# AILab-CVC/SEED-X

Hardware: AMD Instinct MI355X
Metric: end-to-end generations/sec (img-in -> txt + 1024px-img-out) (higher is better)
Workload: dtype fp16

## Files before the change

### include/seedx_hip.h

```cpp
#ifndef SEEDX_HIP_H
#define SEEDX_HIP_H
#include <stdint.h>
#ifdef __cplusplus
extern "C" {
#endif

#define SX_OK 0
#define SX_ERR_INVALID 1
#define SX_ERR_HIP 2

#define SX_F16 0
#define SX_BF16 1
#define SX_F32 2
#define SX_BF16X3 3
#define SX_F16X2 4
#define SX_FP8_E4M3 5
#define SX_FP4_E2M1 6
#define SX_TILED16 0x100

#define SX_ACT_NONE 0
#define SX_ACT_GELU 1
#define SX_ACT_SILU 2

#define SX_A_LINEAR 0
// ... 16 lines not shown
  int32_t bias2d_rows;
  int32_t dtype;
  int32_t out_dtype;
  int32_t act;
  int32_t glu;
  int32_t a_mode;
  int32_t B, Hin, Win, Cin, Hout, Wout;
  int32_t stride;
  int32_t upsample;
  int32_t ld_bias2d;
  int32_t pad_mode;
  int32_t a_planes;
} sx_gemm_args;
int sx_gemm(const sx_gemm_args* args, void* stream);
int sx_gemm_gn(const sx_gemm_args* args, double* stats, int groups, int rows_per_sample, int* fused_host, void* stream);
typedef struct sx_gemm_ln_args {
  void* x16_out;
  double* row_stats_out;
  const double* row_stats_in;
  const float* colsum;
  int32_t ld_x16;
  int32_t dim;
  float eps;
  int32_t reserved;
} sx_gemm_ln_args;
int sx_gemm_ln(const sx_gemm_args* args, const sx_gemm_ln_args* ln, void* stream);
int sx_gemm_force_tile(int cfg);
int sx_gemm_debug_stamps(void* buf);
int sx_gemm_pick_tile(int M, int N, int K, int glu, int conv);

typedef struct sx_gemv_args {
  const void* x;
  const void* W;
  void* y;
  const float* residual;
  int32_t M, N, K;
  int32_t dtype, out_dtype, act, glu;
  int32_t w_layout;
  int32_t x_layout;
// ... 262 lines not shown
```

### seed-x_amd/_lib.py

```python
import ctypes as C
import os

_HERE = os.path.dirname(os.path.abspath(__file__))
LIB_PATH = os.path.join(_HERE, "lib", "libseedx_hip.so")

SX_F16, SX_BF16, SX_F32 = 0, 1, 2
SX_BF16X3 = 3
SX_F16X2 = 4
SX_FP8_E4M3 = 5
SX_FP4_E2M1 = 6
SX_TILED16 = 0x100
SX_ACT_NONE, SX_ACT_GELU, SX_ACT_SILU = 0, 1, 2
SX_A_LINEAR, SX_A_CONV3X3 = 0, 1

c_i32, c_i64, c_f32, c_vp = C.c_int32, C.c_int64, C.c_float, C.c_void_p


class GemmArgs(C.Structure):
    _fields_ = [("A", c_vp), ("W", c_vp), ("C", c_vp), ("bias", c_vp), ("bias2d", c_vp), ("residual", c_vp),
                ("M", c_i32), ("N", c_i32), ("K", c_i32), ("ldc", c_i32), ("ldr", c_i32), ("n_valid", c_i32),
                ("res_mod", c_i32), ("bias2d_rows", c_i32), ("dtype", c_i32), ("out_dtype", c_i32),
                ("act", c_i32), ("glu", c_i32), ("a_mode", c_i32),
                ("B", c_i32), ("Hin", c_i32), ("Win", c_i32), ("Cin", c_i32), ("Hout", c_i32), ("Wout", c_i32),
                ("stride", c_i32), ("upsample", c_i32), ("ld_bias2d", c_i32), ("pad_mode", c_i32), ("a_planes", c_i32)]


class GemmLnArgs(C.Structure):
    _fields_ = [("x16_out", c_vp), ("row_stats_out", c_vp), ("row_stats_in", c_vp), ("colsum", c_vp),
                ("ld_x16", c_i32), ("dim", c_i32), ("eps", c_f32), ("reserved", c_i32)]


class GemvArgs(C.Structure):
    _fields_ = [("x", c_vp), ("W", c_vp), ("y", c_vp), ("residual", c_vp),
                ("M", c_i32), ("N", c_i32), ("K", c_i32),
                ("dtype", c_i32), ("out_dtype", c_i32), ("act", c_i32), ("glu", c_i32),
                ("w_layout", c_i32), ("x_layout", c_i32), ("workspace", c_vp), ("workspace_bytes", C.c_uint64),
                ("x16_out", c_vp), ("row_ssq_out", c_vp), ("row_ssq_in", c_vp), ("ssq_in_parts", c_i32), ("ssq_dim", c_i32),
                ("ssq_eps", c_f32), ("x_planes", c_i32), ("out_planes", c_i32), ("x16_gamma", c_vp),
                ("w_dtype", c_i32), ("w_scale", c_vp), ("w_block_scale", c_vp),
                ("addend", c_vp), ("addend_sel", c_vp), ("addend_n", c_i32)]


class AttnF32Args(C.Structure):
    _fields_ = [("q", c_vp), ("kcache", c_vp), ("vcache", c_vp), ("out", c_vp), ("pos0_dev", c_vp),
# ... 168 lines not shown
```

### seed-x_amd/csrc/gemm.hip

```cpp
#include "gemm_common.h"

namespace sxk_gemm {

template <typename TT, int BM, int BN, int WM, int WN, int NSTAGE, int AMODE>
__global__ __launch_bounds__(WM * WN * 64) void gemm_kernel(const GemmP p) {
#if defined(__HIP_DEVICE_COMPILE__)
  typedef typename TT::vec8 vec8;
  constexpr int NW = WM * WN;
  static_assert(NW == 4 || NW == 8, "4 or 8 waves per block");
  constexpr int TM = BM / WM, TN = BN / WN;
  constexpr int FM = TM / 16, FN = TN / 16;
  constexpr bool kGlu = (FN % 2 == 0);
  constexpr int BNP = (BN + 8 * NW - 1) / (8 * NW) * (8 * NW);
  constexpr int A_PER_WAVE = BM / (8 * NW);
  constexpr int B_PER_WAVE = BNP / (8 * NW);
  constexpr int LOADS = A_PER_WAVE + B_PER_WAVE;
  constexpr int A_BYTES = BM * 128, B_BYTES = BNP * 128, STAGE = A_BYTES + B_BYTES;
  static_assert(LOADS * (NSTAGE - 1) <= 63, "vmcnt range");
  extern __shared__ __attribute__((aligned(16))) unsigned char smem[];

  const int tid = threadIdx.x, lane = tid & 63;
  const int wave = __builtin_amdgcn_readfirstlane(tid >> 6);
  const int wm = wave / WN, wn = wave % WN;
  unsigned long long t_start = 0, t_first = 0, t_main = 0;
// ... 364 lines not shown
  if (gn_fused) *gn_fused = 0;
  SX_CHECK(a->dtype == SX_F16 || a->dtype == SX_BF16, "sx_gemm: dtype must be f16/bf16");
  SX_CHECK(a->out_dtype >= SX_F16 && a->out_dtype <= SX_F32, "sx_gemm: bad out_dtype");
  SX_CHECK(a->M > 0 && a->N > 0 && a->K > 0, "sx_gemm: empty problem M=%d N=%d K=%d", a->M, a->N, a->K);
  SX_CHECK(a->K % 64 == 0, "sx_gemm: K=%d must be a multiple of 64 (pad the operand)", a->K);
  SX_CHECK(a->N % 16 == 0, "sx_gemm: N=%d must be a multiple of 16 (pad the weight)", a->N);
  SX_CHECK(!a->glu || a->N % 32 == 0, "sx_gemm: glu needs N %% 32 == 0");
  const int n_out = a->glu ? a->N / 2 : a->N;
  SX_CHECK(a->n_valid >= 0 && a->n_valid % 4 == 0 && a->n_valid <= n_out, "sx_gemm: n_valid=%d", a->n_valid);
  SX_CHECK(a->ldc >= (a->n_valid > 0 ? a->n_valid : n_out) && a->ldc % 4 == 0, "sx_gemm: ldc=%d invalid for n_out=%d",
           a->ldc, n_out);
  SX_CHECK(!a->residual || (a->ldr >= (a->n_valid > 0 ? a->n_valid : n_out) && a->ldr % 4 == 0), "sx_gemm: ldr=%d invalid", a->ldr);
  SX_CHECK(!a->bias2d || a->bias2d_rows > 0, "sx_gemm: bias2d_rows must be > 0");
  GemmP p;
  memset(&p, 0, sizeof(p));
  p.A = a->A; p.W = a->W; p.C = a->C; p.bias = a->bias; p.bias2d = a->bias2d; p.residual = a->residual;
  SX_CHECK(a->a_planes >= 0 && a->a_planes <= 2, "sx_gemm: a_planes=%d", a->a_planes);
  const int planes = a->a_planes == 2 ? 2 : 1;
  SX_CHECK(planes == 1 || (a->a_mode == SX_A_LINEAR && !ln), "sx_gemm: a_planes = 2 is for plain linear GEMMs");
  const int Kk = a->K * planes;
  p.M = a->M; p.N = a->N; p.K = Kk; p.Kw = a->K; p.ldc = a->ldc; p.ldr = a->ldr; p.res_mod = a->res_mod;
  p.n_valid = a->n_valid > 0 ? a->n_valid : n_out;
  p.bias2d_rows = a->bias2d_rows; p.out_dtype = a->out_dtype; p.act = a->act; p.glu = a->glu;
  p.ldb2 = a->ld_bias2d > 0 ? a->ld_bias2d : a->N;
  p.pad = 1;
  uint64_t a_bytes;
  if (a->a_mode == SX_A_CONV3X3) {
    SX_CHECK(a->Cin % 64 == 0 && a->K == 9 * a->Cin, "sx_gemm conv: Cin=%d K=%d", a->Cin, a->K);
    SX_CHECK(a->stride == 1 || a->stride == 2, "sx_gemm conv: stride");
    SX_CHECK(a->M == a->B * a->Hout * a->Wout, "sx_gemm conv: M != B*Hout*Wout");
// ... 17 lines not shown
  hipStream_t st = (hipStream_t)stream;
  p.res_init = (p.residual && p.act == SX_ACT_NONE && !p.glu) ? 1 : 0;
  if (ln) {
    SX_CHECK(a->a_mode == SX_A_LINEAR && !gn_stats, "sx_gemm_ln: linear GEMMs only");
    SX_CHECK(!(ln->row_stats_in && ln->row_stats_out), "sx_gemm_ln: a launch is a producer or a consumer, not both");
    if (ln->row_stats_out) {
      SX_CHECK(ln->x16_out && a->out_dtype == SX_F32 && !a->glu && a->act == SX_ACT_NONE && p.n_valid == a->N,
               "sx_gemm_ln producer: needs x16_out and a plain fp32 output of all N columns");
      SX_CHECK(ln->ld_x16 >= a->N && ln->ld_x16 % 4 == 0 && (((size_t)ln->x16_out) & 7) == 0, "sx_gemm_ln producer: ld_x16=%d", ln->ld_x16);
      p.ln_x16 = ln->x16_out; p.ln_ldx = ln->ld_x16; p.ln_out = ln->row_stats_out;
    } else {
      SX_CHECK(ln->colsum && ln->dim == a->K && ln->eps > 0.f, "sx_gemm_ln consumer: colsum / dim (= K) / eps");
      SX_CHECK(a->out_dtype == a->dtype && !a->residual && !a->bias2d, "sx_gemm_ln consumer: 16-bit output, no residual / bias2d");
      p.ln_in = ln->row_stats_in; p.ln_cs = ln->colsum; p.ln_eps = ln->eps; p.ln_inv_dim = 1.0f / (float)ln->dim;
    }
  }
  unsigned allow = 0x7f;
  if (ln) allow = 0;
  allow |= pp_supported(p, a->dtype, 256, a->a_mode) ? 0x80u : 0u;
  allow |= pp_supported(p, a->dtype, 320, a->a_mode) ? 0x100u : 0u;
  SX_CHECK(!(g_force_tile == 7 || g_force_tile == 8) || ((allow >> g_force_tile) & 1u),
           "sx_gemm: forced ping-pong tile has no kernel for this epilogue");
  if (ln) {
    const int plain = pick_tile(a->M, a->N, Kk, a->glu != 0, false, g_force_tile, 0x1ff);
    SX_CHECK((plain == 7 || plain == 8) && ((allow >> plain) & 1u),
             "sx_gemm_ln: M=%d N=%d K=%d does not run on a ping-pong tile with this epilogue (tile %d): keep sx_layernorm for it", a->M,
             a->N, a->K, plain);
    allow = 1u << plain;
  }
  const int cfg = pick_tile(a->M, a->N, Kk, a->glu != 0, a->a_mode == SX_A_CONV3X3, g_force_tile, allow);
  if (cfg == 7 || cfg == 8) {
    if (gn_stats && a->out_dtype == SX_F32 && !a->glu && a->act == SX_ACT_NONE && p.n_valid == a->N && a->N % gn_groups == 0 &&
        (a->N / gn_groups) % 2 == 0 && gn_rows % 256 == 0 && a->M % gn_rows == 0) {
      p.gn_stats = gn_stats; p.gn_groups = gn_groups; p.gn_cpg = a->N / gn_groups; p.gn_rows = gn_rows;
      *gn_fused = 1;
    }
    return launch_pp(p, a->dtype, cfg == 7 ? 256 : 320, a->a_mode, st);
  }
#define SX_GEMM_DISPATCH(TT)                                                  \
  switch (cfg) {                                                              \
    case 0: return launch_cfg<TT, 128, 128, 2, 2, 2>(p, a->a_mode, st);       \
    case 1: return launch_cfg<TT, 128, 80, 4, 1, 3>(p, a->a_mode, st);        \
    case 2: return launch_cfg<TT, 64, 128, 2, 2, 3>(p, a->a_mode, st);        \
    case 3: return launch_cfg<TT, 64, 64, 2, 2, 3>(p, a->a_mode, st);         \
    case 4: return launch_cfg<TT, 256, 256, 2, 4, 2>(p, a->a_mode, st);       \
    case 5: return launch_cfg<TT, 256, 320, 2, 4, 2>(p, a->a_mode, st);       \
    default: return launch_cfg<TT, 256, 160, 4, 2, 2>(p, a->a_mode, st);      \
  }
  if (a->dtype == SX_BF16) { SX_GEMM_DISPATCH(BF16) } else { SX_GEMM_DISPATCH(F16) }
#undef SX_GEMM_DISPATCH
}
```

### seed-x_amd/csrc/gemm_common.h

```cpp
#pragma once
#include "sx_common.h"

namespace sxk_gemm {

struct GemmP {
  const void* A;
  const void* W;
  void* C;
  const float* bias;
  const float* bias2d;
  const float* residual;
  int M, N, K, ldc, ldr, n_valid, res_mod, bias2d_rows, out_dtype, act, glu;
  int Kw;
  int Hin, Win, Cin, Hout, Wout, stride, upsample, ldb2, pad;
  int tiles_m, tiles_n, xm, xn;
  int gm;
  int res_init;
  unsigned a_bytes, w_bytes;
  unsigned long long* dbg;
  double* gn_stats;
  int gn_cpg, gn_groups, gn_rows;
  void* ln_x16;
  double* ln_out;
  const double* ln_in;
  const float* ln_cs;
  int ln_ldx;
  float ln_eps, ln_inv_dim;
};

template <int N>
__device__ __forceinline__ void wait_vmcnt() {
  asm volatile("s_waitcnt vmcnt(%0)" ::"n"(N) : "memory");
}

__device__ __forceinline__ bool tile_coords(const GemmP& p, int bid, int nblk, int& tile_m, int& tile_n) {
  if (p.xm == 0) {
    const int t = xcd_remap(bid, nblk);
    tile_m = t % p.tiles_m;
    tile_n = t / p.tiles_m;
    return true;
  }
  const int xcd = bid & 7, idx = bid >> 3;
// ... 21 lines not shown
    const double ab = (double)p.M * p.K, wb = (double)p.N * p.K;
    double best = 1e300;
    for (int xm = 1; xm <= 8; xm *= 2) {
      const int xn = 8 / xm;
      if (xm > p.tiles_m || xn > p.tiles_n) continue;
      const long padded = 8L * ((p.tiles_m + xm - 1) / xm) * ((p.tiles_n + xn - 1) / xn);
      const double cost = (ab * xn + wb * xm) * (1.0 + 4.0 * (double)(padded - grid) / grid);
      if (cost < best) { best = cost; p.xm = xm; p.xn = xn; }
    }
    if (p.xm) grid = 8 * ((p.tiles_m + p.xm - 1) / p.xm) * ((p.tiles_n + p.xn - 1) / p.xn);
    p.gm = gm_force > 0 ? gm_force : 8;
  }
  return grid;
}

int launch_pp(const GemmP& p, int dtype, int bn, int a_mode, hipStream_t st);
bool pp_supported(const GemmP& p, int dtype, int bn, int a_mode);

extern unsigned long long* g_dbg;
extern int g_gm;
extern int g_xcd_2d;

}
```

### seed-x_amd/csrc/gemm_pp.hip

```cpp
#include "gemm_common.h"
#include <type_traits>

namespace sxk_gemm {

#define SX_A_CONV3X3_UP 2

#define PP_SYNC()                            \
  do {                                       \
    __builtin_amdgcn_sched_barrier(0);       \
    __builtin_amdgcn_s_barrier();            \
    __builtin_amdgcn_sched_barrier(0);       \
  } while (0)

template <typename TT, int BN, int AMODE, bool OUT32, int ACT, bool GLU, int LN = 0>
__global__ __launch_bounds__(512) void gemm_pp_kernel(const GemmP p) {
#if defined(__HIP_DEVICE_COMPILE__)
  typedef typename TT::vec8 vec8;
  static_assert(LN != 2 || (OUT32 && !GLU && ACT == SX_ACT_NONE), "the LayerNorm producer is the plain fp32-output epilogue");
  constexpr int BM = 256, TN = BN / 4, FN = TN / 16, FM = 8, FH = 4;
  constexpr int NB = BN / 64;
  constexpr int C1 = NB - 3, C2 = 3;
  constexpr int WAITN = 4 + NB;
  constexpr int A_BYTES = BM * 128, STAGE = A_BYTES + BN * 128;
  static_assert(!GLU || FN % 2 == 0, "GLU pairs n-fragments");
  static_assert(BN == 256 || BN == 320, "ping-pong tiles are 256x256 and 256x320");
  extern __shared__ __attribute__((aligned(16))) unsigned char smem[];

  const int tid = threadIdx.x, lane = tid & 63;
  const int wave = __builtin_amdgcn_readfirstlane(tid >> 6);
  const int g = wave >> 2, wc = wave & 3;
// ... 199 lines not shown
    wait_vmcnt<WAITN>();
    lgkm0();
    PP_SYNC();
    mma(wf1, 1);
    PP_SYNC();
  };

  for (int kt = 0; kt < nkt; kt += 2) {
    ktile(std::integral_constant<int, 0>{}, kt);
    if (kt + 1 < nkt) ktile(std::integral_constant<int, 1>{}, kt + 1);
  }
  if (g == 0) PP_SYNC();
  wait_vmcnt<0>();

  if (p.dbg) t_main = __builtin_amdgcn_s_memtime();
  int ncol[FN], nout[FN];
  bool nok[FN];
  f32x4_t bv[FN];
#pragma unroll
  for (int i = 0; i < FN; ++i) {
    const int nb = n0 + wc * TN + i * 16;
    ncol[i] = nb + lq;
    nout[i] = GLU ? (nb >> 1) + lq : ncol[i];
    nok[i] = ncol[i] < p.N && nout[i] < p.n_valid && !(GLU && (i & 1));
    if (ncol[i] >= p.N) ncol[i] = p.N - 4;
    if (nout[i] + 4 > p.ldc) nout[i] = 0;
    bv[i] = (f32x4_t){0.f, 0.f, 0.f, 0.f};
  }
  if (p.bias) {
#pragma unroll
// ... 216 lines not shown
      for (int cp = c_lo >> 1; cp < (c_hi >> 1); ++cp) acc += gslot[((size_t)(BN / 2) + cp) * 2 + which];
      atomicAdd(&p.gn_stats[((size_t)smp * p.gn_groups + G) * 2 + which], (double)acc);
    }
  }
  if (p.dbg) {
    asm volatile("s_waitcnt vmcnt(0)" ::: "memory");
    const unsigned long long t_end = __builtin_amdgcn_s_memtime();
    if (tid == 0) {
      unsigned long long* d = p.dbg + (size_t)blockIdx.x * 4;
      d[0] = t_start; d[1] = t_first; d[2] = t_main; d[3] = t_end;
    }
  }
#endif
}

template <typename TT, int BN, int AMODE, bool OUT32, int ACT, bool GLU, int LN = 0>
static int launch_one(const GemmP& p0, hipStream_t st) {
  GemmP p = p0;
  p.dbg = g_dbg;
  const int grid = plan_grid(p, 256, BN, g_xcd_2d, g_gm);
  constexpr size_t lds = 2 * (size_t)(256 + BN) * 128 + (LN == 1 ? 2048 : 0);
  auto k = gemm_pp_kernel<TT, BN, AMODE, OUT32, ACT, GLU, LN>;
  static hipError_t attr[16];
  static bool done[16];
  int dev = 0;
  (void)hipGetDevice(&dev);
  dev &= 15;
  if (!done[dev]) {
    attr[dev] = hipFuncSetAttribute((const void*)k, hipFuncAttributeMaxDynamicSharedMemorySize, (int)lds);
    done[dev] = true;
  }
  SX_CHECK(attr[dev] == hipSuccess, "sx_gemm: cannot reserve %zu B of LDS for the 256x%d ping-pong tile: %s", lds, BN,
           hipGetErrorString(attr[dev]));
  hipLaunchKernelGGL(k, dim3(grid), dim3(512), lds, st, p);
  SX_HIP_LAUNCH_CHECK();
  return SX_OK;
}

static int epi_code(const GemmP& p, int dtype) {
  const bool out32 = p.out_dtype == SX_F32;
  if (!out32 && p.out_dtype != dtype) return -1;
  if (p.glu) {
    if (out32) return -1;
    if (p.act == SX_ACT_GELU) return 2;
    if (p.act == SX_ACT_SILU) return 3;
    return -1;
  }
  if (p.act == SX_ACT_NONE) return out32 ? 4 : 0;
  if (p.act == SX_ACT_GELU && !out32) return 1;
  return -1;
}

bool pp_supported(const GemmP& p, int dtype, int bn, int a_mode) {
  const int e = epi_code(p, dtype);
  if (e < 0) return false;
  if (p.ln_in && !(a_mode == SX_A_LINEAR && (e == 0 || e == 2) && !p.ln_out)) return false;
  if (p.ln_out && !(a_mode == SX_A_LINEAR && e == 4 && !p.gn_stats)) return false;
  if (bn == 320 && (e == 2 || e == 3)) return false;
  if (a_mode == SX_A_CONV3X3 && !(e == 0 || e == 4)) return false;
  if (a_mode == SX_A_CONV3X3 && p.upsample && !(p.stride == 1 && p.pad == 1)) return false;
  return bn == 256 || bn == 320;
}

template <typename TT>
static int launch_t(const GemmP& p, int dtype, int bn, int a_mode, hipStream_t st) {
  const int e = epi_code(p, dtype);
#define PP_CASE(BNV, AM, O32, ACTV, GLUV) return launch_one<TT, BNV, AM, O32, ACTV, GLUV>(p, st)
  if (p.ln_in) {
    if (e == 2) return launch_one<TT, 256, SX_A_LINEAR, false, SX_ACT_GELU, true, 1>(p, st);
    if (bn == 256) return launch_one<TT, 256, SX_A_LINEAR, false, SX_ACT_NONE, false, 1>(p, st);
    return launch_one<TT, 320, SX_A_LINEAR, false, SX_ACT_NONE, false, 1>(p, st);
  }
  if (p.ln_out) {
    if (bn == 256) return launch_one<TT, 256, SX_A_LINEAR, true, SX_ACT_NONE, false, 2>(p, st);
    return launch_one<TT, 320, SX_A_LINEAR, true, SX_ACT_NONE, false, 2>(p, st);
  }
  if (a_mode == SX_A_LINEAR) {
    if (bn == 256) {
      switch (e) {
        case 0: PP_CASE(256, SX_A_LINEAR, false, SX_ACT_NONE, false);
        case 1: PP_CASE(256, SX_A_LINEAR, false, SX_ACT_GELU, false);
        case 2: PP_CASE(256, SX_A_LINEAR, false, SX_ACT_GELU, true);
        case 3: PP_CASE(256, SX_A_LINEAR, false, SX_ACT_SILU, true);
        case 4: PP_CASE(256, SX_A_LINEAR, true, SX_ACT_NONE, false);
      }
// ... 21 lines not shown
      switch (e) {
        case 0: PP_CASE(256, SX_A_CONV3X3_UP, false, SX_ACT_NONE, false);
        case 4: PP_CASE(256, SX_A_CONV3X3_UP, true, SX_ACT_NONE, false);
      }
    } else {
      switch (e) {
        case 0: PP_CASE(320, SX_A_CONV3X3_UP, false, SX_ACT_NONE, false);
        case 4: PP_CASE(320, SX_A_CONV3X3_UP, true, SX_ACT_NONE, false);
      }
    }
  }
#undef PP_CASE
  return -1;
}

int launch_pp(const GemmP& p, int dtype, int bn, int a_mode, hipStream_t st) {
  if (!pp_supported(p, dtype, bn, a_mode)) return -1;
  return dtype == SX_BF16 ? launch_t<BF16>(p, dtype, bn, a_mode, st) : launch_t<F16>(p, dtype, bn, a_mode, st);
}

}
```

### seed-x_amd/ops.py

```python
import ctypes as C
import math

import os

import torch

from . import _lib
from ._lib import (SX_A_CONV3X3, SX_A_LINEAR, SX_ACT_GELU, SX_ACT_NONE, SX_ACT_SILU, SX_BF16, SX_F16, SX_F32,
                   AttnArgs, AttnSmallArgs, GemmArgs, GemvArgs, check)

_DT = {torch.float16: SX_F16, torch.bfloat16: SX_BF16, torch.float32: SX_F32}
_TD = {v: k for k, v in _DT.items()}
ACT = {None: SX_ACT_NONE, "none": SX_ACT_NONE, "gelu": SX_ACT_GELU, "silu": SX_ACT_SILU}


def dt_code(dtype):
    return _DT[dtype]


def _stream():
    return C.c_void_p(torch.cuda.current_stream().cuda_stream)


def _p(t):
# ... 34 lines not shown
def gemm_tile(M, N, K, glu=False, conv=False):
    return int(_lib.load().sx_gemm_pick_tile(int(M), int(N), int(K), 1 if glu else 0, 1 if conv else 0))


def ln_fold_ok(M, C, consumers, producers):
    return all(gemm_tile(M, n, C, glu) >= 7 for n, glu in consumers) and all(gemm_tile(M, C, k) >= 7 for k in producers)


def fold_layernorm(w, bias, gamma, beta):
    wf = (w.float() * gamma.float()[None, :]).to(w.dtype).contiguous()
    cs = wf.float().sum(dim=1).contiguous()
    b = w.float() @ beta.float()
    if bias is not None:
        b = b + bias.float()
    return wf, cs, b.contiguous()


GN_FUSE = os.environ.get("SX_GN_FUSE", "1") != "0"


def _launch_gemm(lib, args, gn, what):
    if gn is None or not GN_FUSE:
        check(lib.sx_gemm(C.byref(args), _stream()), what)
        return
    assert gn.buf.dtype == torch.float64 and gn.buf.is_contiguous() and args.M % gn.rows == 0 \
        and gn.buf.numel() == (args.M // gn.rows) * gn.groups * 2, "GnStats does not describe this output"
    fused = C.c_int32(0)
    check(lib.sx_gemm_gn(C.byref(args), gn.buf.data_ptr(), gn.groups, gn.rows, C.byref(fused), _stream()), what)
    gn.ready = bool(fused.value)


def gemm(a, w, bias=None, bias2d=None, bias2d_rows=0, residual=None, res_mod=0, act=None, glu=False,
         out_dtype=None, out=None, n_valid=0, ld_bias2d=0, gn=None, ln_emit=None, ln_apply=None, a_planes=1):
    lib = _lib.load()
    assert a.dim() == 2 and w.dim() == 2 and a.is_contiguous() and w.is_contiguous()
    assert a.dtype == w.dtype and a.dtype in (torch.float16, torch.bfloat16)
    M, K = a.shape
    N = w.shape[0]
    assert a_planes in (1, 2) and K % a_planes == 0
    K //= a_planes
    assert w.shape[1] == K, f"K mismatch {a.shape} vs {w.shape} (a_planes {a_planes})"
    n_out = N // 2 if glu else N
    n_store = n_valid if n_valid else n_out
    out_dtype = out_dtype or a.dtype
    if out is None:
        out = torch.empty((M, n_store), dtype=out_dtype, device=a.device)
    assert out.dtype == out_dtype and out.stride(-1) == 1 and out.shape[0] == M
    args = GemmArgs()
# ... 16 lines not shown
    args.out_dtype = _DT[out_dtype]
    args.act = ACT[act]
    args.glu = 1 if glu else 0
    args.a_mode = SX_A_LINEAR
    args.a_planes = a_planes
    if ln_emit is not None or ln_apply is not None:
        assert gn is None and not (ln_emit is not None and ln_apply is not None)
        la = _lib.GemmLnArgs()
        if ln_emit is not None:
            assert ln_emit.x16.shape == (M, N) and ln_emit.x16.dtype == a.dtype and ln_emit.stats.shape[0] == M
            la.x16_out, la.ld_x16, la.row_stats_out = ln_emit.x16.data_ptr(), ln_emit.x16.stride(0), ln_emit.stats.data_ptr()
        else:
            rows, colsum, eps = ln_apply
            assert rows.stats.shape[0] == M and colsum.dtype == torch.float32 and colsum.numel() == N and colsum.is_contiguous()
            la.row_stats_in, la.colsum, la.dim, la.eps = rows.stats.data_ptr(), colsum.data_ptr(), K, float(eps)
        check(lib.sx_gemm_ln(C.byref(args), C.byref(la), _stream()), "sx_gemm_ln")
        return out
    _launch_gemm(lib, args, gn, "sx_gemm")
    return out


def conv3x3(x, w, bias=None, bias2d=None, residual=None, stride=1, upsample=False, out_dtype=None, act=None,
            n_valid=0, pad_mode=0, gn=None):
    lib = _lib.load()
    assert x.dim() == 4 and x.is_contiguous() and w.is_contiguous()
    B, H, W, Cin = x.shape
    Cout, K = w.shape
    assert K == 9 * Cin
    hv, wv = (2 * H, 2 * W) if upsample else (H, W)
    padsum = 1 if pad_mode else 2
    Hout, Wout = (hv + padsum - 3) // stride + 1, (wv + padsum - 3) // stride + 1
    M = B * Hout * Wout
# ... 842 lines not shown
```

### seed-x_amd/unet.py

```python
import math
import os
import types

import torch

from . import ops
from .llama import glu_pack_rows

LN_FOLD = os.environ.get("SX_LN_FOLD", "1") != "0"

SDXL_BASE_CONFIG = dict(in_channels=4, out_channels=4, block_out_channels=(320, 640, 1280), layers_per_block=2,
                        down_attn=(False, True, True), up_attn=(True, True, False), transformer_layers=(1, 2, 10),
                        heads=(5, 10, 20), cross_attention_dim=2048, addition_time_embed_dim=256, pooled_dim=1280,
                        norm_groups=32, sample_size=128)


class UNetOutput:
    def __init__(self, sample):
        self.sample = sample


class UNet2DConditionModel:
    def __init__(self, comm=None, **cfg):
        from .parallel import Comm
# ... 133 lines not shown
                    wqkv=torch.cat([lin16(b + f".attn1.{q}.weight") for q in ("to_q", "to_k", "to_v")], 0).contiguous(),
                    wo1=lin16(b + ".attn1.to_out.0.weight"), bo1=f32(b + ".attn1.to_out.0.bias"),
                    n2=(f32(b + ".norm2.weight"), f32(b + ".norm2.bias")),
                    wq2=lin16(b + ".attn2.to_q.weight"),
                    wkv2=torch.cat([lin16(b + ".attn2.to_k.weight"), lin16(b + ".attn2.to_v.weight")], 0).contiguous(),
                    wo2=lin16(b + ".attn2.to_out.0.weight"), bo2=f32(b + ".attn2.to_out.0.bias"),
                    n3=(f32(b + ".norm3.weight"), f32(b + ".norm3.bias")),
                    wff1=glu_pack_rows(ffw[:half].contiguous(), ffw[half:].contiguous()),
                    bff1=glu_pack_rows(ffb[:half].reshape(-1, 1).contiguous(), ffb[half:].reshape(-1, 1).contiguous()).reshape(-1).contiguous(),
                    wff2=lin16(b + ".ff.net.2.weight"), bff2=f32(b + ".ff.net.2.bias")))
            if LN_FOLD:
                for blk in t["blocks"]:
                    blk["f1"] = ops.fold_layernorm(blk["wqkv"], None, *blk["n1"])
                    blk["f2"] = ops.fold_layernorm(blk["wq2"], None, *blk["n2"])
                    blk["f3"] = ops.fold_layernorm(blk["wff1"], blk["bff1"], *blk["n3"])
            self._xattn.append(t)
            return t

        self._temb_names, self._xattn = [], []
        boc = c["block_out_channels"]
        P = {}
        cin = c["in_channels"]
        self.cin_kpad = (9 * cin + 63) // 64 * 64
        w = sd["conv_in.weight"].detach().to(dev, dt).permute(0, 2, 3, 1).reshape(boc[0], -1)
        wp = torch.zeros(boc[0], self.cin_kpad, dtype=dt, device=dev)
        wp[:, :w.shape[1]] = w
        P["conv_in_w"], P["conv_in_b"] = wp, f32("conv_in.bias")
        P["te1"] = (lin16("time_embedding.linear_1.weight"), f32("time_embedding.linear_1.bias"))
        P["te2"] = (lin16("time_embedding.linear_2.weight"), f32("time_embedding.linear_2.bias"))
        P["ae1"] = (lin16("add_embedding.linear_1.weight"), f32("add_embedding.linear_1.bias"))
# ... 101 lines not shown
    def _transformer(self, t, x, B, ctx_kv, Hc, Wc, st_in=None):
        dt, heads = self.dtype, t["heads"]
        _, HW, C = x.shape
        hd = C // heads
        scale = hd ** -0.5
        sp = self.comm.world > 1
        h = self._gn(x, t["norm"], 1e-6, False, Hc, Wc, stats=st_in)
        nb = len(t["blocks"])
        M = B * HW
        if LN_FOLD and not sp and "f1" in t["blocks"][0] and self._ln_fold_ok(M, C):
            arena = torch.zeros((3 * nb, M, 2), dtype=torch.float64, device=x.device)

            def rows(i):
                return ops.LnRows(M, C, dt, x.device, stats=arena[i])
            ln = rows(0)
            hs = ops.gemm(h.view(-1, C), t["pin_w"], bias=t["pin_b"], out_dtype=torch.float32, ln_emit=ln)
            for k, b in enumerate(t["blocks"]):
                w, cs, bb = b["f1"]
                qkv = ops.gemm(ln.x16, w, bias=bb, ln_apply=(ln, cs, 1e-5)).view(B, HW, 3, heads, hd)
                att = ops.attention(qkv[:, :, 0], qkv[:, :, 1], qkv[:, :, 2], scale)
                ln = rows(3 * k + 1)
                hs = ops.gemm(att.view(-1, C), b["wo1"], bias=b["bo1"], residual=hs, out_dtype=torch.float32, ln_emit=ln)
                self._mark(hs)
                w, cs, bb = b["f2"]
                q = ops.gemm(ln.x16, w, bias=bb, ln_apply=(ln, cs, 1e-5)).view(B, HW, heads, hd)
                kv = ctx_kv[k]
                att = ops.attention(q, kv[:, :, 0], kv[:, :, 1], scale)
                ln = rows(3 * k + 2)
                hs = ops.gemm(att.view(-1, C), b["wo2"], bias=b["bo2"], residual=hs, out_dtype=torch.float32, ln_emit=ln)
                w, cs, bb = b["f3"]
                g = ops.gemm(ln.x16, w, bias=bb, act="gelu", glu=True, ln_apply=(ln, cs, 1e-5))
                if k == nb - 1:
                    hs = ops.gemm(g, b["wff2"], bias=b["bff2"], residual=hs, out_dtype=dt)
                else:
                    ln = rows(3 * k + 3)
                    hs = ops.gemm(g, b["wff2"], bias=b["bff2"], residual=hs, out_dtype=torch.float32, ln_emit=ln)
                self._mark(hs)
            st_out = self._gn_slot(B, HW)
            out = ops.gemm(hs, t["pout_w"], bias=t["pout_b"], residual=x.view(-1, C), out_dtype=torch.float32, gn=st_out)
            return out.view(B, HW, C), st_out
        hs = ops.gemm(h.view(-1, C), t["pin_w"], bias=t["pin_b"], out_dtype=torch.float32)
        for k, b in enumerate(t["blocks"]):
# ... 1 lines not shown
            if not sp:
                qkv = ops.gemm(n, b["wqkv"]).view(B, HW, 3, heads, hd)
                att = ops.attention(qkv[:, :, 0], qkv[:, :, 1], qkv[:, :, 2], scale)
            else:
                from . import seqpar
                kv_l = ops.gemm(n, b["wqkv"][C:]).view(B, HW, 2, heads, hd)
                pending = self.comm.all_gather_async(kv_l)
                q = ops.gemm(n, b["wqkv"][:C]).view(B, HW, heads, hd)
                g = pending.wait()
                kv = g.permute(1, 0, 2, 3, 4, 5).reshape(B, g.shape[0] * HW, 2, heads, hd).contiguous()
                att = ops.attention(q, kv[:, :, 0], kv[:, :, 1], scale)
            hs = ops.gemm(att.view(-1, C), b["wo1"], bias=b["bo1"], residual=hs, out_dtype=torch.float32)
            self._mark(hs)
            n = ops.layernorm(hs, b["n2"][0], b["n2"][1], 1e-5, dt)
            q = ops.gemm(n, b["wq2"]).view(B, HW, heads, hd)
            kv = ctx_kv[k]
            att = ops.attention(q, kv[:, :, 0], kv[:, :, 1], scale)
            hs = ops.gemm(att.view(-1, C), b["wo2"], bias=b["bo2"], residual=hs, out_dtype=torch.float32)
            n = ops.layernorm(hs, b["n3"][0], b["n3"][1], 1e-5, dt)
            g = ops.gemm(n, b["wff1"], bias=b["bff1"], act="gelu", glu=True)
            last = k == nb - 1
            hs = ops.gemm(g, b["wff2"], bias=b["bff2"], residual=hs, out_dtype=dt if last else torch.float32)
            self._mark(hs)
        st_out = self._gn_slot(B, HW)
        out = ops.gemm(hs, t["pout_w"], bias=t["pout_b"], residual=x.view(-1, C), out_dtype=torch.float32, gn=st_out)
        return out.view(B, HW, C), st_out

    def _ln_fold_ok(self, M, C):
        key = (M, C)
        if key not in self._ln_ok:
            self._ln_ok[key] = ops.ln_fold_ok(M, C, consumers=[(3 * C, False), (C, False), (8 * C, True)], producers=[C, 4 * C])
        return self._ln_ok[key]

    def prepare_context(self, encoder_hidden_states):
        P = self._pack()
        ehs = encoder_hidden_states
        key = (ehs.data_ptr(), ehs._version, tuple(ehs.shape))
        if self._ctx_key == key:
            return self._ctx
        B, L, ca = ehs.shape
        e16 = ops.cast(ehs.to(self.device).float().contiguous(), self.dtype).view(B * L, ca)
        ctx = []
        for t in self._xattn:
            heads = t["heads"]
            per = []
            for b in t["blocks"]:
                C = b["wq2"].shape[0]
                kv = ops.gemm(e16, b["wkv2"]).view(B, L, 2, heads, C // heads)
                per.append(kv)
            ctx.append(per)
        self._ctx_key, self._ctx = key, ctx
        return ctx

    def time_embeddings(self, t_vals, idx_dev, text_embeds, time_ids, B):
        P, dt, c = self._P, self.dtype, self.cfg
        boc0 = c["block_out_channels"][0]
        ts = ops.timestep_embedding(t_vals, boc0, dt, idx_dev=idx_dev, n=B)
        e = ops.gemm(ts, P["te1"][0], bias=P["te1"][1], act="silu")
        e = ops.gemm(e, P["te2"][0], bias=P["te2"][1], out_dtype=torch.float32)
        tid = ops.timestep_embedding(time_ids.reshape(-1).float().contiguous(), c["addition_time_embed_dim"], torch.float32)
        add = torch.empty((B, self.add_embedding.linear_1.in_features), dtype=torch.float32, device=self.device)
        ops.copy2d(text_embeds.float().contiguous(), add, 0)
        ops.copy2d(tid.view(B, -1), add, text_embeds.shape[1])
# ... 88 lines not shown
```

Baseline: 1.343.

## Fuse cross-attention into the LayerNorm-folded Q-projection GEMM epilogue

Adds an epilogue variant to the 320-wide ping-pong GEMM that, after computing the Q projection with folded LayerNorm, loads pre-packed K/V fragments for a 64-token context into LDS and runs softmax attention with MFMA directly on the register tile, writing the attention output. Q-projection weight columns are permuted so each wave owns whole heads (with a fifth head shared via LDS). Context K/V is additionally packed into an MFMA fragment layout once per context. This removes the Q write/read round trip and the separate attention launch per transformer block, at the cost of tight shape constraints (head_dim 64, 64 context tokens, heads multiple of 5) and heavier epilogue work per tile.

```diff
diff --git a/include/seedx_hip.h b/include/seedx_hip.h
--- a/include/seedx_hip.h
+++ b/include/seedx_hip.h
@@ -54,6 +54,15 @@
 } sx_gemm_args;
 int sx_gemm(const sx_gemm_args* args, void* stream);
 int sx_gemm_gn(const sx_gemm_args* args, double* stats, int groups, int rows_per_sample, int* fused_host, void* stream);
+typedef struct sx_xattn_args {
+  const void* kv_frag;
+  void* O;
+  int32_t heads, head_dim, skv;
+  int32_t rows_per_sample;
+  int32_t ld_o;
+  int32_t ld_kv;
+  float scale;
+} sx_xattn_args;
 typedef struct sx_gemm_ln_args {
   void* x16_out;
   double* row_stats_out;
@@ -63,6 +72,7 @@
   int32_t dim;
   float eps;
   int32_t reserved;
+  const void* xattn;
 } sx_gemm_ln_args;
 int sx_gemm_ln(const sx_gemm_args* args, const sx_gemm_ln_args* ln, void* stream);
 int sx_gemm_force_tile(int cfg);
diff --git a/seed-x_amd/_lib.py b/seed-x_amd/_lib.py
--- a/seed-x_amd/_lib.py
+++ b/seed-x_amd/_lib.py
@@ -25,9 +25,14 @@
                 ("stride", c_i32), ("upsample", c_i32), ("ld_bias2d", c_i32), ("pad_mode", c_i32), ("a_planes", c_i32)]
 
 
+class XattnArgs(C.Structure):
+    _fields_ = [("kv_frag", c_vp), ("O", c_vp), ("heads", c_i32), ("head_dim", c_i32), ("skv", c_i32),
+                ("rows_per_sample", c_i32), ("ld_o", c_i32), ("ld_kv", c_i32), ("scale", c_f32)]
+
+
 class GemmLnArgs(C.Structure):
     _fields_ = [("x16_out", c_vp), ("row_stats_out", c_vp), ("row_stats_in", c_vp), ("colsum", c_vp),
-                ("ld_x16", c_i32), ("dim", c_i32), ("eps", c_f32), ("reserved", c_i32)]
+                ("ld_x16", c_i32), ("dim", c_i32), ("eps", c_f32), ("reserved", c_i32), ("xattn", c_vp)]
 
 
 class GemvArgs(C.Structure):
diff --git a/seed-x_amd/csrc/gemm.hip b/seed-x_amd/csrc/gemm.hip
--- a/seed-x_amd/csrc/gemm.hip
+++ b/seed-x_amd/csrc/gemm.hip
@@ -402,6 +402,9 @@
   SX_CHECK(!a->bias2d || a->bias2d_rows > 0, "sx_gemm: bias2d_rows must be > 0");
   GemmP p;
   memset(&p, 0, sizeof(p));
+  XattnP xp;
+  const XattnP* xpp = nullptr;
+  memset(&xp, 0, sizeof(xp));
   p.A = a->A; p.W = a->W; p.C = a->C; p.bias = a->bias; p.bias2d = a->bias2d; p.residual = a->residual;
   SX_CHECK(a->a_planes >= 0 && a->a_planes <= 2, "sx_gemm: a_planes=%d", a->a_planes);
   const int planes = a->a_planes == 2 ? 2 : 1;
@@ -449,11 +452,30 @@
       SX_CHECK(a->out_dtype == a->dtype && !a->residual && !a->bias2d, "sx_gemm_ln consumer: 16-bit output, no residual / bias2d");
       p.ln_in = ln->row_stats_in; p.ln_cs = ln->colsum; p.ln_eps = ln->eps; p.ln_inv_dim = 1.0f / (float)ln->dim;
     }
+    if (const sx_xattn_args* xa = (const sx_xattn_args*)ln->xattn) {
+      SX_CHECK(ln->row_stats_in, "sx_gemm_ln: xattn rides on the consumer launch");
+      SX_CHECK(xa->kv_frag && xa->O && xa->scale > 0.f, "sx_gemm_ln xattn: kv_frag / O / scale");
+      SX_CHECK(xa->head_dim == 64 && xa->skv == 64, "sx_gemm_ln xattn: head_dim=%d skv=%d (64 / 64 only)", xa->head_dim, xa->skv);
+      SX_CHECK(xa->heads > 0 && xa->heads % 5 == 0 && a->N == 64 * xa->heads, "sx_gemm_ln xattn: heads=%d N=%d (heads %% 5 == 0, N = 64 heads)",
+               xa->heads, a->N);
+      SX_CHECK(xa->rows_per_sample > 0 && xa->rows_per_sample % 256 == 0 && a->M % xa->rows_per_sample == 0,
+               "sx_gemm_ln xattn: rows_per_sample=%d M=%d (whole 256-row tiles inside one sample)", xa->rows_per_sample, a->M);
+      SX_CHECK(a->act == SX_ACT_NONE && !a->glu && p.n_valid == a->N, "sx_gemm_ln xattn: plain projection only");
+      SX_CHECK(xa->ld_o >= a->N && xa->ld_o % 8 == 0 && (((size_t)xa->O) & 15) == 0 && (((size_t)xa->kv_frag) & 15) == 0,
+               "sx_gemm_ln xattn: ld_o=%d / alignment", xa->ld_o);
+      SX_CHECK(xa->ld_kv >= xa->heads * 8192 && xa->ld_kv % 8 == 0, "sx_gemm_ln xattn: ld_kv=%d", xa->ld_kv);
+      const uint64_t kv_bytes = (uint64_t)(a->M / xa->rows_per_sample - 1) * xa->ld_kv * 2ull + (uint64_t)xa->heads * 16384ull;
+      SX_CHECK(kv_bytes < 0x7fffffffull, "sx_gemm_ln xattn: packed K | V exceeds the 2 GiB descriptor range");
+      xp.kv = xa->kv_frag; xp.O = xa->O; xp.kv_bytes = (unsigned)kv_bytes; xp.heads = xa->heads;
+      xp.sample_bytes = (unsigned)xa->ld_kv * 2u;
+      xp.rows = xa->rows_per_sample; xp.ldo = xa->ld_o; xp.scale_log2 = xa->scale * 1.4426950408889634f;
+      xpp = &xp;
+    }
   }
   unsigned allow = 0x7f;
   if (ln) allow = 0;
-  allow |= pp_supported(p, a->dtype, 256, a->a_mode) ? 0x80u : 0u;
-  allow |= pp_supported(p, a->dtype, 320, a->a_mode) ? 0x100u : 0u;
+  allow |= pp_supported(p, a->dtype, 256, a->a_mode, xpp) ? 0x80u : 0u;
+  allow |= pp_supported(p, a->dtype, 320, a->a_mode, xpp) ? 0x100u : 0u;
   SX_CHECK(!(g_force_tile == 7 || g_force_tile == 8) || ((allow >> g_force_tile) & 1u),
            "sx_gemm: forced ping-pong tile has no kernel for this epilogue");
   if (ln) {
@@ -470,7 +492,7 @@
       p.gn_stats = gn_stats; p.gn_groups = gn_groups; p.gn_cpg = a->N / gn_groups; p.gn_rows = gn_rows;
       *gn_fused = 1;
     }
-    return launch_pp(p, a->dtype, cfg == 7 ? 256 : 320, a->a_mode, st);
+    return launch_pp(p, a->dtype, cfg == 7 ? 256 : 320, a->a_mode, st, xpp);
   }
 #define SX_GEMM_DISPATCH(TT)                                                  \
   switch (cfg) {                                                              \
diff --git a/seed-x_amd/csrc/gemm_common.h b/seed-x_amd/csrc/gemm_common.h
--- a/seed-x_amd/csrc/gemm_common.h
+++ b/seed-x_amd/csrc/gemm_common.h
@@ -26,6 +26,18 @@
   const float* ln_cs;
   int ln_ldx;
   float ln_eps, ln_inv_dim;
+};
+
+struct XattnP {
+  const void* kv;
+  void* O;
+  unsigned kv_bytes;
+  int heads, rows, ldo;
+  unsigned sample_bytes;
+  float scale_log2;
+};
+struct GemmPX : GemmP {
+  XattnP xa;
 };
 
 template <int N>
@@ -77,8 +89,8 @@
   return grid;
 }
 
-int launch_pp(const GemmP& p, int dtype, int bn, int a_mode, hipStream_t st);
-bool pp_supported(const GemmP& p, int dtype, int bn, int a_mode);
+int launch_pp(const GemmP& p, int dtype, int bn, int a_mode, hipStream_t st, const XattnP* xa = nullptr);
+bool pp_supported(const GemmP& p, int dtype, int bn, int a_mode, const XattnP* xa = nullptr);
 
 extern unsigned long long* g_dbg;
 extern int g_gm;
diff --git a/seed-x_amd/csrc/gemm_pp.hip b/seed-x_amd/csrc/gemm_pp.hip
--- a/seed-x_amd/csrc/gemm_pp.hip
+++ b/seed-x_amd/csrc/gemm_pp.hip
@@ -12,8 +12,8 @@
     __builtin_amdgcn_sched_barrier(0);       \
   } while (0)
 
-template <typename TT, int BN, int AMODE, bool OUT32, int ACT, bool GLU, int LN = 0>
-__global__ __launch_bounds__(512) void gemm_pp_kernel(const GemmP p) {
+template <typename TT, int BN, int AMODE, bool OUT32, int ACT, bool GLU, int LN = 0, bool XA = false>
+__global__ __launch_bounds__(512) void gemm_pp_kernel(const std::conditional_t<XA, GemmPX, GemmP> p) {
 #if defined(__HIP_DEVICE_COMPILE__)
   typedef typename TT::vec8 vec8;
   static_assert(LN != 2 || (OUT32 && !GLU && ACT == SX_ACT_NONE), "the LayerNorm producer is the plain fp32-output epilogue");
@@ -243,6 +243,154 @@
   wait_vmcnt<0>();
 
   if (p.dbg) t_main = __builtin_amdgcn_s_memtime();
+  if constexpr (XA) {
+    static_assert(BN == 320 && LN == 1 && !OUT32 && !GLU && ACT == SX_ACT_NONE && AMODE == SX_A_LINEAR, "cross-attention epilogue");
+    constexpr unsigned HEAD_B = 16384, Q5_OFF = 5 * HEAD_B, XB_OFF = Q5_OFF + 256 * 128, XC_OFF = XB_OFF + 2048;
+    static_assert(XC_OFF + 2048 <= 2 * STAGE, "K | V^T fragments, the fifth head's Q and the column vectors fit in the operand ring");
+    __syncthreads();
+    {
+      __amdgpu_buffer_rsrc_t rKV = __builtin_amdgcn_make_buffer_rsrc((void*)p.xa.kv, 0, (int)p.xa.kv_bytes, 0x00020000);
+      const unsigned kv0 = (unsigned)(m0 / p.xa.rows) * p.xa.sample_bytes + (unsigned)(5 * tile_n) * HEAD_B + (unsigned)lane * 16u;
+#pragma unroll
+      for (int i = 0; i < 10; ++i) {
+        const unsigned c = (unsigned)(wave * 10 + i) * 1024u;
+        __builtin_amdgcn_raw_ptr_buffer_load_lds(rKV, SX_LDS_PTR(smem + c), 16, kv0 + c, 0, 0, 0);
+      }
+      if (wave < 4) {
+        const float* src = wave < 2 ? p.bias : p.ln_cs;
+        __amdgpu_buffer_rsrc_t rV = __builtin_amdgcn_make_buffer_rsrc((void*)src, 0, src ? p.N * 4 : 0, 0x00020000);
+        const unsigned c = (unsigned)(wave & 1) * 1024u;
+        __builtin_amdgcn_raw_ptr_buffer_load_lds(rV, SX_LDS_PTR(smem + (wave < 2 ? XB_OFF : XC_OFF) + c), 16,
+                                                 (unsigned)n0 * 4u + c + (unsigned)lane * 16u, 0, 0, 0);
+      }
+    }
+    auto pack4x = [&](f32x4_t x) -> u32x2_t {
+      u32x2_t o;
+      o[0] = pack2<TT>(x[0], x[1]);
+      o[1] = pack2<TT>(x[2], x[3]);
+      return o;
+    };
+    const int q4 = lane >> 4, r16 = lane & 15;
+    f32x4_t xb[FN], xc[FN];
+    {
+      const int col = n0 + wc * TN + (FN - 1) * 16 + lq;
+      xb[FN - 1] = p.bias ? *(const f32x4_t*)(p.bias + col) : (f32x4_t){0.f, 0.f, 0.f, 0.f};
+      xc[FN - 1] = *(const f32x4_t*)(p.ln_cs + col);
+    }
+    const int row0 = g * 128 + r16;
+    const unsigned char* lnb = (const unsigned char*)ln_lds + row0 * 8;
+    unsigned char* q5w = smem + Q5_OFF + row0 * 128 + (wc * 16 + lq) * 2;
+#pragma unroll
+    for (int j = 0; j < FM; ++j) {
+      const f32x2_t ab = *(const f32x2_t*)(lnb + j * 128);
+      const f32x4_t v = acc[FN - 1][j] * ab[0] + (xc[FN - 1] * ab[1] + xb[FN - 1]);
+      *(u32x2_t*)(q5w + j * 2048) = pack4x(v);
+    }
+    wait_vmcnt<0>();
+    __syncthreads();
+    vec8 kfr[8];
+    const unsigned char* vbase = smem;
+    auto load_kv = [&](int hh) {
+      const unsigned char* base = smem + hh * HEAD_B + lane * 16;
+#pragma unroll
+      for (int f = 0; f < 8; ++f) kfr[f] = *(const vec8*)(base + f * 1024);
+      vbase = base + 8192;
+    };
+    const float cs2 = p.xa.scale_log2;
+    unsigned short* Ob = (unsigned short*)p.xa.O;
+    auto attend = [&](const vec8 (&qb)[2], int m, int head) {
+      f32x4_t s[4];
+#pragma unroll
+      for (int kf = 0; kf < 4; ++kf) {
+        s[kf] = TT::mfma16(kfr[2 * kf], qb[0], (f32x4_t){0.f, 0.f, 0.f, 0.f});
+        s[kf] = TT::mfma16(kfr[2 * kf + 1], qb[1], s[kf]);
+      }
+      float mx = fmaxf(fmaxf(s[0][0], s[0][1]), fmaxf(s[0][2], s[0][3]));
+#pragma unroll
+      for (int kf = 1; kf < 4; ++kf) mx = fmaxf(mx, fmaxf(fmaxf(s[kf][0], s[kf][1]), fmaxf(s[kf][2], s[kf][3])));
+      mx = fmaxf(mx, __shfl_xor(mx, 16, 64));
+      mx = fmaxf(mx, __shfl_xor(mx, 32, 64));
+      const float mc = -mx * cs2;
+      u32x2_t pw[4];
+      float l = 0.f;
+#pragma unroll
+      for (int kf = 0; kf < 4; ++kf) {
+        f32x4_t e;
+#pragma unroll
+        for (int r = 0; r < 4; ++r) e[r] = __builtin_amdgcn_exp2f(__builtin_fmaf(s[kf][r], cs2, mc));
+        pw[kf] = pack4x(e);
+        l = TT::pair_sum(pw[kf][0], l);
+        l = TT::pair_sum(pw[kf][1], l);
+      }
+      l += __shfl_xor(l, 16, 64);
+      l += __shfl_xor(l, 32, 64);
+      const float inv = l > 0.f ? 1.0f / l : 0.f;
+      vec8 pb[2];
+#pragma unroll
+      for (int s2 = 0; s2 < 2; ++s2) {
+        const u32x4_t w = {pw[2 * s2][0], pw[2 * s2][1], pw[2 * s2 + 1][0], pw[2 * s2 + 1][1]};
+        pb[s2] = __builtin_bit_cast(vec8, w);
+      }
+      f32x4_t o[4];
+#pragma unroll
+      for (int df = 0; df < 4; ++df) {
+        o[df] = TT::mfma16(*(const vec8*)(vbase + 2 * df * 1024), pb[0], (f32x4_t){0.f, 0.f, 0.f, 0.f});
+        o[df] = TT::mfma16(*(const vec8*)(vbase + (2 * df + 1) * 1024), pb[1], o[df]);
+      }
+#pragma unroll
+      for (int k = 0; k < 2; ++k) {
+        const u32x2_t o0 = pack4x(o[2 * k] * inv), o1 = pack4x(o[2 * k + 1] * inv);
+        const auto s0 = __builtin_amdgcn_permlane16_swap(o0[0], o1[0], false, false);
+        const auto s1 = __builtin_amdgcn_permlane16_swap(o0[1], o1[1], false, false);
+        const u32x4_t w4 = {s0[0], s1[0], s0[1], s1[1]};
+        const int col = head * 64 + k * 32 + (q4 & 1) * 16 + (q4 >> 1) * 8;
+        *(u32x4_t*)(Ob + (size_t)m * p.xa.ldo + col) = w4;
+      }
+    };
+    load_kv(4);
+#pragma unroll
+    for (int jj = 0; jj < 2; ++jj) {
+      const int row = wave * 32 + jj * 16 + r16;
+      const unsigned char* qr = smem + Q5_OFF + row * 128 + lq * 2;
+      vec8 qb[2];
+#pragma unroll
+      for (int s2 = 0; s2 < 2; ++s2) {
+        const u32x2_t lo = *(const u32x2_t*)(qr + s2 * 64), hi = *(const u32x2_t*)(qr + s2 * 64 + 32);
+        const u32x4_t w = {lo[0], lo[1], hi[0], hi[1]};
+        qb[s2] = __builtin_bit_cast(vec8, w);
+      }
+      attend(qb, m0 + row, 5 * tile_n + 4);
+    }
+    load_kv(wc);
+#pragma unroll
+    for (int i = 0; i < 4; ++i) {
+      xb[i] = *(const f32x4_t*)(smem + XB_OFF + (wc * TN + i * 16 + lq) * 4);
+      xc[i] = *(const f32x4_t*)(smem + XC_OFF + (wc * TN + i * 16 + lq) * 4);
+    }
+#pragma unroll
+    for (int j = 0; j < FM; ++j) {
+      const f32x2_t ab = *(const f32x2_t*)(lnb + j * 128);
+      u32x2_t qw[4];
+#pragma unroll
+      for (int i = 0; i < 4; ++i) qw[i] = pack4x(acc[i][j] * ab[0] + (xc[i] * ab[1] + xb[i]));
+      vec8 qb[2];
+#pragma unroll
+      for (int s2 = 0; s2 < 2; ++s2) {
+        const u32x4_t w = {qw[2 * s2][0], qw[2 * s2][1], qw[2 * s2 + 1][0], qw[2 * s2 + 1][1]};
+        qb[s2] = __builtin_bit_cast(vec8, w);
+      }
+      attend(qb, m0 + row0 + j * 16, 5 * tile_n + wc);
+    }
+    if (p.dbg) {
+      asm volatile("s_waitcnt vmcnt(0)" ::: "memory");
+      const unsigned long long t_end = __builtin_amdgcn_s_memtime();
+      if (tid == 0) {
+        unsigned long long* d = p.dbg + (size_t)blockIdx.x * 4;
+        d[0] = t_start; d[1] = t_first; d[2] = t_main; d[3] = t_end;
+      }
+    }
+    return;
+  }
   int ncol[FN], nout[FN];
   bool nok[FN];
   f32x4_t bv[FN];
@@ -489,13 +637,15 @@
 #endif
 }
 
-template <typename TT, int BN, int AMODE, bool OUT32, int ACT, bool GLU, int LN = 0>
-static int launch_one(const GemmP& p0, hipStream_t st) {
-  GemmP p = p0;
+template <typename TT, int BN, int AMODE, bool OUT32, int ACT, bool GLU, int LN = 0, bool XA = false>
+static int launch_one(const GemmP& p0, hipStream_t st, const XattnP* xa = nullptr) {
+  std::conditional_t<XA, GemmPX, GemmP> p;
+  static_cast<GemmP&>(p) = p0;
+  if constexpr (XA) p.xa = *xa;
   p.dbg = g_dbg;
   const int grid = plan_grid(p, 256, BN, g_xcd_2d, g_gm);
   constexpr size_t lds = 2 * (size_t)(256 + BN) * 128 + (LN == 1 ? 2048 : 0);
-  auto k = gemm_pp_kernel<TT, BN, AMODE, OUT32, ACT, GLU, LN>;
+  auto k = gemm_pp_kernel<TT, BN, AMODE, OUT32, ACT, GLU, LN, XA>;
   static hipError_t attr[16];
   static bool done[16];
   int dev = 0;
@@ -526,10 +676,11 @@
   return -1;
 }
 
-bool pp_supported(const GemmP& p, int dtype, int bn, int a_mode) {
+bool pp_supported(const GemmP& p, int dtype, int bn, int a_mode, const XattnP* xa) {
   const int e = epi_code(p, dtype);
   if (e < 0) return false;
   if (p.ln_in && !(a_mode == SX_A_LINEAR && (e == 0 || e == 2) && !p.ln_out)) return false;
+  if (xa && !(p.ln_in && e == 0 && bn == 320)) return false;
   if (p.ln_out && !(a_mode == SX_A_LINEAR && e == 4 && !p.gn_stats)) return false;
   if (bn == 320 && (e == 2 || e == 3)) return false;
   if (a_mode == SX_A_CONV3X3 && !(e == 0 || e == 4)) return false;
@@ -538,12 +689,13 @@
 }
 
 template <typename TT>
-static int launch_t(const GemmP& p, int dtype, int bn, int a_mode, hipStream_t st) {
+static int launch_t(const GemmP& p, int dtype, int bn, int a_mode, hipStream_t st, const XattnP* xa) {
   const int e = epi_code(p, dtype);
 #define PP_CASE(BNV, AM, O32, ACTV, GLUV) return launch_one<TT, BNV, AM, O32, ACTV, GLUV>(p, st)
   if (p.ln_in) {
     if (e == 2) return launch_one<TT, 256, SX_A_LINEAR, false, SX_ACT_GELU, true, 1>(p, st);
     if (bn == 256) return launch_one<TT, 256, SX_A_LINEAR, false, SX_ACT_NONE, false, 1>(p, st);
+    if (xa) return launch_one<TT, 320, SX_A_LINEAR, false, SX_ACT_NONE, false, 1, true>(p, st, xa);
     return launch_one<TT, 320, SX_A_LINEAR, false, SX_ACT_NONE, false, 1>(p, st);
   }
   if (p.ln_out) {
@@ -595,9 +747,9 @@
   return -1;
 }
 
-int launch_pp(const GemmP& p, int dtype, int bn, int a_mode, hipStream_t st) {
-  if (!pp_supported(p, dtype, bn, a_mode)) return -1;
-  return dtype == SX_BF16 ? launch_t<BF16>(p, dtype, bn, a_mode, st) : launch_t<F16>(p, dtype, bn, a_mode, st);
+int launch_pp(const GemmP& p, int dtype, int bn, int a_mode, hipStream_t st, const XattnP* xa) {
+  if (!pp_supported(p, dtype, bn, a_mode, xa)) return -1;
+  return dtype == SX_BF16 ? launch_t<BF16>(p, dtype, bn, a_mode, st, xa) : launch_t<F16>(p, dtype, bn, a_mode, st, xa);
 }
 
 }
diff --git a/seed-x_amd/ops.py b/seed-x_amd/ops.py
--- a/seed-x_amd/ops.py
+++ b/seed-x_amd/ops.py
@@ -72,6 +72,56 @@
     if bias is not None:
         b = b + bias.float()
     return wf, cs, b.contiguous()
+
+
+XATTN_D = 64
+
+
+def xattn_fuse_ok(M, C, heads, rows_per_sample, skv):
+    return (heads > 0 and heads % 5 == 0 and C == XATTN_D * heads and skv == XATTN_D and rows_per_sample > 0
+            and rows_per_sample % 256 == 0 and M % rows_per_sample == 0 and gemm_tile(M, C, C) == 8)
+
+
+def xattn_col_perm(heads):
+    assert heads % 5 == 0
+    pos = torch.arange(XATTN_D * heads)
+    t, wc, i, c = pos // 320, (pos % 320) // 80, (pos % 80) // 16, pos % 16
+    own = i < 4
+    head = 5 * t + torch.where(own, wc, torch.full_like(wc, 4))
+    d = torch.where(own, 16 * i, 16 * wc) + c
+    return head * XATTN_D + d
+
+
+def _xattn_frag_index():
+    f, l, e = torch.arange(8)[:, None, None], torch.arange(64)[None, :, None], torch.arange(8)[None, None, :]
+    slot = 32 * (f % 2) + 16 * (e // 4) + 4 * (l // 16) + (e % 4)
+    row = 16 * (f // 2) + (l % 16) + 0 * e
+    return row, slot, slot, row
+
+
+def pack_xattn_kv(kv):
+    B, L, two, heads, D = kv.shape
+    assert L == XATTN_D and D == XATTN_D and two == 2
+    kk, kd, vk, vd = (x.to(kv.device) for x in _xattn_frag_index())
+    k, v = kv[:, :, 0].permute(0, 2, 1, 3), kv[:, :, 1].permute(0, 2, 1, 3)
+    return torch.stack([k[:, :, kk, kd], v[:, :, vk, vd]], dim=2).contiguous()
+
+
+def unpack_xattn_kv(frag):
+    B, heads = frag.shape[:2]
+    kk, kd, vk, vd = (x.to(frag.device) for x in _xattn_frag_index())
+    k = torch.empty((B, heads, XATTN_D, XATTN_D), dtype=frag.dtype, device=frag.device)
+    v = torch.empty_like(k)
+    k[:, :, kk, kd] = frag[:, :, 0]
+    v[:, :, vk, vd] = frag[:, :, 1]
+    return torch.stack([k.permute(0, 2, 1, 3), v.permute(0, 2, 1, 3)], dim=2).contiguous()
+
+
+class Xattn:
+    __slots__ = ("kv_frag", "scale", "rows_per_sample")
+
+    def __init__(self, kv_frag, scale, rows_per_sample):
+        self.kv_frag, self.scale, self.rows_per_sample = kv_frag, float(scale), int(rows_per_sample)
 
 
 GN_FUSE = os.environ.get("SX_GN_FUSE", "1") != "0"
@@ -89,7 +139,7 @@
 
 
 def gemm(a, w, bias=None, bias2d=None, bias2d_rows=0, residual=None, res_mod=0, act=None, glu=False,
-         out_dtype=None, out=None, n_valid=0, ld_bias2d=0, gn=None, ln_emit=None, ln_apply=None, a_planes=1):
+         out_dtype=None, out=None, n_valid=0, ld_bias2d=0, gn=None, ln_emit=None, ln_apply=None, a_planes=1, xattn=None):
     lib = _lib.load()
     assert a.dim() == 2 and w.dim() == 2 and a.is_contiguous() and w.is_contiguous()
     assert a.dtype == w.dtype and a.dtype in (torch.float16, torch.bfloat16)
@@ -136,8 +186,18 @@
             rows, colsum, eps = ln_apply
             assert rows.stats.shape[0] == M and colsum.dtype == torch.float32 and colsum.numel() == N and colsum.is_contiguous()
             la.row_stats_in, la.colsum, la.dim, la.eps = rows.stats.data_ptr(), colsum.data_ptr(), K, float(eps)
+        if xattn is not None:
+            assert ln_apply is not None, "xattn rides on the LayerNorm consumer launch"
+            f = xattn.kv_frag
+            assert f.dtype == a.dtype and f.dim() == 6 and tuple(f.shape[2:]) == (2, 8, 64, 8) and f[0].is_contiguous()
+            assert f.shape[0] * xattn.rows_per_sample == M, "one packed context per sample"
+            xa = _lib.XattnArgs()
+            xa.kv_frag, xa.O, xa.ld_o, xa.ld_kv = f.data_ptr(), out.data_ptr(), out.stride(0), f.stride(0)
+            xa.heads, xa.head_dim, xa.skv, xa.rows_per_sample, xa.scale = f.shape[1], XATTN_D, XATTN_D, xattn.rows_per_sample, xattn.scale
+            la.xattn = C.cast(C.pointer(xa), C.c_void_p)
         check(lib.sx_gemm_ln(C.byref(args), C.byref(la), _stream()), "sx_gemm_ln")
         return out
+    assert xattn is None, "xattn rides on the LayerNorm consumer launch (ln_apply)"
     _launch_gemm(lib, args, gn, "sx_gemm")
     return out
 
diff --git a/seed-x_amd/unet.py b/seed-x_amd/unet.py
--- a/seed-x_amd/unet.py
+++ b/seed-x_amd/unet.py
@@ -8,6 +8,7 @@
 from .llama import glu_pack_rows
 
 LN_FOLD = os.environ.get("SX_LN_FOLD", "1") != "0"
+XATTN_FUSE = os.environ.get("SX_XATTN_FUSE", "1") != "0"
 
 SDXL_BASE_CONFIG = dict(in_channels=4, out_channels=4, block_out_channels=(320, 640, 1280), layers_per_block=2,
                         down_attn=(False, True, True), up_attn=(True, True, False), transformer_layers=(1, 2, 10),
@@ -171,6 +172,9 @@
                     blk["f1"] = ops.fold_layernorm(blk["wqkv"], None, *blk["n1"])
                     blk["f2"] = ops.fold_layernorm(blk["wq2"], None, *blk["n2"])
                     blk["f3"] = ops.fold_layernorm(blk["wff1"], blk["bff1"], *blk["n3"])
+                    if XATTN_FUSE and heads % 5 == 0 and blk["wq2"].shape[0] == ops.XATTN_D * heads:
+                        perm = ops.xattn_col_perm(heads).to(dev)
+                        blk["f2x"] = tuple(x[perm].contiguous() for x in blk["f2"])
             self._xattn.append(t)
             return t
 
@@ -302,6 +306,8 @@
             def rows(i):
                 return ops.LnRows(M, C, dt, x.device, stats=arena[i])
             ln = rows(0)
+            fuse = (XATTN_FUSE and "f2x" in t["blocks"][0] and ctx_kv[0].dim() == 3 and ctx_kv[0].shape[0] == B
+                    and ops.xattn_fuse_ok(M, C, heads, HW, ops.XATTN_D))
             hs = ops.gemm(h.view(-1, C), t["pin_w"], bias=t["pin_b"], out_dtype=torch.float32, ln_emit=ln)
             for k, b in enumerate(t["blocks"]):
                 w, cs, bb = b["f1"]
@@ -310,10 +316,14 @@
                 ln = rows(3 * k + 1)
                 hs = ops.gemm(att.view(-1, C), b["wo1"], bias=b["bo1"], residual=hs, out_dtype=torch.float32, ln_emit=ln)
                 self._mark(hs)
-                w, cs, bb = b["f2"]
-                q = ops.gemm(ln.x16, w, bias=bb, ln_apply=(ln, cs, 1e-5)).view(B, HW, heads, hd)
-                kv = ctx_kv[k]
-                att = ops.attention(q, kv[:, :, 0], kv[:, :, 1], scale)
+                kv, frag = self._ctx_planes(ctx_kv[k], heads, hd)
+                if fuse:
+                    w, cs, bb = b["f2x"]
+                    att = ops.gemm(ln.x16, w, bias=bb, ln_apply=(ln, cs, 1e-5), xattn=ops.Xattn(frag, scale, HW))
+                else:
+                    w, cs, bb = b["f2"]
+                    q = ops.gemm(ln.x16, w, bias=bb, ln_apply=(ln, cs, 1e-5)).view(B, HW, heads, hd)
+                    att = ops.attention(q, kv[:, :, 0], kv[:, :, 1], scale)
                 ln = rows(3 * k + 2)
                 hs = ops.gemm(att.view(-1, C), b["wo2"], bias=b["bo2"], residual=hs, out_dtype=torch.float32, ln_emit=ln)
                 w, cs, bb = b["f3"]
@@ -345,7 +355,7 @@
             self._mark(hs)
             n = ops.layernorm(hs, b["n2"][0], b["n2"][1], 1e-5, dt)
             q = ops.gemm(n, b["wq2"]).view(B, HW, heads, hd)
-            kv = ctx_kv[k]
+            kv, _ = self._ctx_planes(ctx_kv[k], heads, hd)
             att = ops.attention(q, kv[:, :, 0], kv[:, :, 1], scale)
             hs = ops.gemm(att.view(-1, C), b["wo2"], bias=b["bo2"], residual=hs, out_dtype=torch.float32)
             n = ops.layernorm(hs, b["n3"][0], b["n3"][1], 1e-5, dt)
@@ -356,6 +366,13 @@
         st_out = self._gn_slot(B, HW)
         out = ops.gemm(hs, t["pout_w"], bias=t["pout_b"], residual=x.view(-1, C), out_dtype=torch.float32, gn=st_out)
         return out.view(B, HW, C), st_out
+
+    @staticmethod
+    def _ctx_planes(c, heads, hd):
+        if c.dim() == 5:
+            return c, None
+        B = c.shape[0]
+        return c[:, 0].view(B, -1, 2, heads, hd), c[:, 1].view(B, heads, 2, 8, 64, 8)
 
     def _ln_fold_ok(self, M, C):
         key = (M, C)
@@ -378,6 +395,11 @@
             for b in t["blocks"]:
                 C = b["wq2"].shape[0]
                 kv = ops.gemm(e16, b["wkv2"]).view(B, L, 2, heads, C // heads)
+                if "f2x" in b and L == ops.XATTN_D:
+                    both = torch.empty((B, 2, 2 * L * C), dtype=kv.dtype, device=kv.device)
+                    both[:, 0] = kv.reshape(B, -1)
+                    both[:, 1] = ops.pack_xattn_kv(kv).reshape(B, -1)
+                    kv = both
                 per.append(kv)
             ctx.append(per)
         self._ctx_key, self._ctx = key, ctx
```

Result: no change. 1.350 (median of 6 runs) (+0.6%).
